# kamenbliznashki/chexpert

Measured on AMD Instinct MI355X. Metric: images/sec fwd+bwd DenseNet121 320x320 bf16 (per-GPU rate in config.images_per_sec_per_gpu), higher is better.
Workload: dtype bf16; 1 GPU; densenet121 bf16 1xMI355X 320x320 bs=256 per GPU, U-Ones labels (BASELINE configs[1]); 14 classes; random-init weights, synthetic uint8 X-rays; per_gpu_batch=256, global_batch=256, parallelism=dp1, rccl_ranks=1, capture_failed=0, launch=hipGraph replay

## Files before the change

### chexpert_amd/csrc/conv_gemm.hip

```cpp
#include "common.h"

namespace {

constexpr int BM = 128;
constexpr int BK = 32;
constexpr int PITCH = 80;
constexpr int A_BYTES = BM * PITCH;

template <int BN>
struct Geo {
  static constexpr int WAVES_N = (BN >= 64) ? 2 : 1;
  static constexpr int WAVES_M = 4 / WAVES_N;
  static constexpr int TM = BM / (WAVES_M * 32);
  static constexpr int TN = BN / (WAVES_N * 32);
  static constexpr int B_BYTES = BN * PITCH;
  static constexpr int STAGE = A_BYTES + B_BYTES;
  static constexpr int EPITCH = BN + 4;
  static constexpr int EPI_BYTES = 64 * EPITCH * 4;
  static constexpr int MAIN_BYTES = (2 * STAGE > EPI_BYTES) ? 2 * STAGE : EPI_BYTES;
};

template <int PRO>
struct NCoef {
  static constexpr int v = (PRO == CX_PRO_NONE) ? 0 : (PRO == CX_PRO_AFFINE_RELU ? 2 : 3);
};

template <int BN, int PRO, int MODE, int EPI>
__global__ __launch_bounds__(256) void conv_gemm_kernel(const CxConv p, const int M, const int n_tiles) {
  using G = Geo<BN>;
  constexpr int NSRC = (MODE == CX_MODE_POOL2) ? 4 : 1;
  extern __shared__ __attribute__((aligned(16))) char smem[];
  float* coef = reinterpret_cast<float*>(smem);
  char* tiles = smem + NCoef<PRO>::v * p.K * 4;

  const int tid = threadIdx.x;
  const int lane = tid & 63;
  const int wave = tid >> 6;
  const int wm = wave / G::WAVES_N, wn = wave % G::WAVES_N;
  const int wgid = xcd_remap(blockIdx.x, gridDim.x);
  const int mt = wgid / n_tiles, nt = wgid % n_tiles;
  const int n0 = nt * BN;

  if (PRO != CX_PRO_NONE) {
    for (int i = tid; i < p.K; i += 256) {
      coef[i] = p.pa[i];
      coef[p.K + i] = p.pb[i];
      if (PRO == CX_PRO_AFFINE2) coef[2 * p.K + i] = p.pc[i];
    }
  }

  const int qa = tid & 3;
  int rb[2], riy[2], rix[2];
  bool rvalid[2];
#pragma unroll
  for (int i = 0; i < 2; ++i) {
    const int m = mt * BM + (tid >> 2) + 64 * i;
    rvalid[i] = m < M;
    const int mm = rvalid[i] ? m : 0;
    const int hw = p.Ho * p.Wo;
    rb[i] = mm / hw;
    const int rem = mm - rb[i] * hw;
    const int oy = rem / p.Wo, ox = rem - oy * p.Wo;
    if (MODE == CX_MODE_CONV) {
      riy[i] = oy * p.stride - p.pad;
      rix[i] = ox * p.stride - p.pad;
    } else if (MODE == CX_MODE_POOL2) {
      riy[i] = 2 * oy;
      rix[i] = 2 * ox;
    } else {
      riy[i] = 2 * oy - 3;
      rix[i] = 2 * ox - 4 + 2 * qa;
    }
  }
  const int kpt = (MODE == CX_MODE_STEM) ? 1 : (p.K + BK - 1) / BK;
  const int taps = (MODE == CX_MODE_STEM) ? 7 : p.kh * p.kw;
  const int nsteps = taps * kpt;
  const bf16* __restrict__ X = reinterpret_cast<const bf16*>(p.x);
  const bf16* __restrict__ X2 = reinterpret_cast<const bf16*>(p.x2);
  const bf16* __restrict__ Wp = reinterpret_cast<const bf16*>(p.w);

  uint4 ra[2][NSRC], ra2[2], rbw[2];
  bool av[2], wv[2] = {false, false};

  const int ts_sh = p.tstride > 1 ? 1 : 0;
  const int cdil = p.dil > 1 ? p.dil : 1;
  int q_tap = 0, q_kc = 0, q_dy = 0, q_dx = 0, w_kc = 0;
  auto issue_loads = [&](int s) {
    (void)s;
    const int tap = q_tap, kc = q_kc;
    const int dy = (MODE == CX_MODE_CONV) ? q_dy * cdil : tap;
    const int dx = (MODE == CX_MODE_CONV) ? q_dx * cdil : 0;
    w_kc = kc;
#pragma unroll
    for (int i = 0; i < 2; ++i) {
      if (MODE == CX_MODE_STEM) {
        const int iy = riy[i] + dy, ix = rix[i];
        av[i] = rvalid[i] & (iy >= 0) & (iy < p.H) & (ix >= 0) & (ix < p.W);
        const int cy = av[i] ? iy : 0, cx = av[i] ? ix : 0;
        ra[i][0] = *reinterpret_cast<const uint4*>(X + ((size_t)(rb[i] * p.H + cy) * p.W + cx) * 4);
      } else if (MODE == CX_MODE_POOL2) {
        av[i] = rvalid[i];
#pragma unroll
        for (int a = 0; a < 4; ++a) {
          const size_t pix = (size_t)(rb[i] * p.H + riy[i] + (a >> 1)) * p.W + rix[i] + (a & 1);
          ra[i][a] = *reinterpret_cast<const uint4*>(X + pix * p.ldx + kc * BK + qa * 8);
        }
      } else {
        int iy = riy[i] + dy, ix = rix[i] + dx;
        bool ok = rvalid[i] & (iy >= 0) & (ix >= 0) & (((iy | ix) & ts_sh) == 0);
        iy >>= ts_sh;
        ix >>= ts_sh;
        const bool kok = kc * BK + qa * 8 < p.K;
// ... 32 lines not shown
    const int tap = 0, kc = w_kc;
    char* A = tiles + buf * G::STAGE;
    char* Bt = A + A_BYTES;
    const int c0 = kc * BK + qa * 8;
#pragma unroll
    for (int i = 0; i < 2; ++i) {
      U128 o;
      if (!av[i]) {
        o.u = make_uint4(0, 0, 0, 0);
      } else if (PRO == CX_PRO_NONE) {
        o.u = ra[i][0];
      } else if (PRO == CX_PRO_AFFINE_RELU) {
        float acc[8];
#pragma unroll
        for (int j = 0; j < 8; ++j) acc[j] = 0.f;
#pragma unroll
        for (int a = 0; a < NSRC; ++a) {
          const uint32_t w4[4] = {ra[i][a].x, ra[i][a].y, ra[i][a].z, ra[i][a].w};
#pragma unroll
          for (int j = 0; j < 4; ++j) {
            acc[2 * j] += fmaxf(fmaf(cx_bf_lo(w4[j]), coef[c0 + 2 * j], coef[p.K + c0 + 2 * j]), 0.f);
            acc[2 * j + 1] += fmaxf(fmaf(cx_bf_hi(w4[j]), coef[c0 + 2 * j + 1], coef[p.K + c0 + 2 * j + 1]), 0.f);
          }
        }
        {
          const float sc_ = NSRC == 4 ? 0.25f : 1.f;
          o.u = make_uint4(cx_packbf(acc[0] * sc_, acc[1] * sc_), cx_packbf(acc[2] * sc_, acc[3] * sc_), cx_packbf(acc[4] * sc_, acc[5] * sc_),
                           cx_packbf(acc[6] * sc_, acc[7] * sc_));
        }
      } else {
        o.u = cx_affine2_8(ra[i][0], ra2[i], coef + c0, coef + p.K + c0, coef + 2 * p.K + c0);
      }
      *reinterpret_cast<uint4*>(A + ((tid >> 2) + 64 * i) * PITCH + qa * 16) = o.u;
    }
#pragma unroll
    for (int i = 0; i < 2; ++i) {
      const int nb = (tid >> 2) + 64 * i;
      if (nb < BN) *reinterpret_cast<uint4*>(Bt + nb * PITCH + qa * 16) = wv[i] ? rbw[i] : make_uint4(0, 0, 0, 0);
    }
    (void)tap;
  };

  f32x16 acc[G::TM][G::TN];
#pragma unroll
  for (int i = 0; i < G::TM; ++i)
#pragma unroll
    for (int j = 0; j < G::TN; ++j)
#pragma unroll
      for (int r = 0; r < 16; ++r) acc[i][j][r] = 0.f;

  issue_loads(0);
  __syncthreads();
  write_stage(0, 0);
  __syncthreads();

  const int lrow = lane & 31, lh = lane >> 5;
  for (int s = 0; s < nsteps; ++s) {
    const int buf = s & 1;
    if (s + 1 < nsteps) issue_loads(s + 1);
    const char* A = tiles + buf * G::STAGE;
    const char* Bt = A + A_BYTES;
#pragma unroll
    for (int kk = 0; kk < 2; ++kk) {
      bf16x8 af[G::TM], bfr[G::TN];
#pragma unroll
      for (int i = 0; i < G::TM; ++i)
// ... 107 lines not shown
            const float du = (fmaf(xu, esc[2 * j + 1], esh[2 * j + 1]) > 0.f) ? v[2 * j + 1] : 0.f;
            s1[2 * j] += dl;
            s1[2 * j + 1] += du;
            s2[2 * j] += dl * (xl - emu[2 * j]) * er[2 * j];
            s2[2 * j + 1] += du * (xu - emu[2 * j + 1]) * er[2 * j + 1];
            w4[j] = cx_packbf(fmaf(escale[2 * j], dl, cx_bf_lo(ow[j])), fmaf(escale[2 * j + 1], du, cx_bf_hi(ow[j])));
          }
          o.u = make_uint4(w4[0], w4[1], w4[2], w4[3]);
        }
        *reinterpret_cast<uint4*>(Y + (size_t)m * p.ldy + nch) = o.u;
      }
    }
    __syncthreads();
  }

  if (want_stats) {
#pragma unroll
    for (int j = 0; j < 8; ++j) {
#pragma unroll
      for (int d = CPR; d < 64; d <<= 1) {
        s1[j] += __shfl_xor(s1[j], d);
        s2[j] += __shfl_xor(s2[j], d);
      }
    }
    float* scratch = reinterpret_cast<float*>(tiles);
    wg_stat_begin<4>(scratch, BN, tid, 256);
    if (lane < CPR) {
#pragma unroll
      for (int j = 0; j < 8; ++j) wg_stat_put(scratch, BN, wave, cq * 8 + j, s1[j], s2[j]);
    }
    wg_stat_end<4>(scratch, BN, tid, 256, p.stat_sum, p.stat_sq, p.stat_det, p.stat_det ? mt : (int)blockIdx.x, p.stat_replicas,
                   p.stat_rstride, n0, p.N);
  }
}

template <int BN, int PRO, int MODE, int EPI>
int launch(const CxConv& p, hipStream_t st) {
  using G = Geo<BN>;
  const long long M = (long long)p.B * p.Ho * p.Wo;
  const int m_tiles = (int)((M + BM - 1) / BM);
  const int n_tiles = (p.N + BN - 1) / BN;
  const size_t smem = (size_t)NCoef<PRO>::v * p.K * 4 + G::MAIN_BYTES + 2 * BN * 4;
  if (smem > 160 * 1024) return CX_ESHAPE;
  if (const int e = stat_rows_check(p, m_tiles)) return e;
  static bool attr_set = false;
  if (!attr_set && smem > 64 * 1024) {
    (void)hipFuncSetAttribute(reinterpret_cast<const void*>(&conv_gemm_kernel<BN, PRO, MODE, EPI>),
                        hipFuncAttributeMaxDynamicSharedMemorySize, 160 * 1024);
    attr_set = true;
  }
  CX_KTAG("conv_gemm_kernel<%d, %d, %d, %d>", BN, PRO, MODE, EPI);
  hipLaunchKernelGGL((conv_gemm_kernel<BN, PRO, MODE, EPI>), dim3(m_tiles * n_tiles), dim3(256), smem, st, p, (int)M,
                     n_tiles);
  return launch_status();
}

template <int PRO, int MODE, int EPI>
int launch_bn(const CxConv& p, hipStream_t st) {
  if (p.N % 128 == 0) return launch<128, PRO, MODE, EPI>(p, st);
  if (p.N == 32) return launch<32, PRO, MODE, EPI>(p, st);
  return launch<64, PRO, MODE, EPI>(p, st);
}

}

int cx_try_pc_fwd(const CxConv& p, hipStream_t st, bool* handled);
int cx_try_ring_fwd(const CxConv& p, hipStream_t st, bool* handled);
int cx_try_strip_fwd(const CxConv& p, hipStream_t st, bool* handled);
int cx_try_ring_dgrad(const CxConv& p, hipStream_t st, bool* handled);
int cx_try_strip_dgrad(const CxConv& p, hipStream_t st, bool* handled);
int cx_try_pw_dgrad(const CxConv& p, hipStream_t st, bool* handled);
int cx_try_pw_fwd(const CxConv& p, hipStream_t st, bool* handled);
int cx_try_pw_fwdk(const CxConv& p, hipStream_t st, bool* handled);
int cx_try_pw_xs(const CxConv& p, hipStream_t st, bool* handled);
int cx_try_stem_fwd(const CxConv& p, hipStream_t st, bool* handled);
int cx_conv_gemm_f32(const CxConv& p, hipStream_t st);
int cx_try_conv_mm(const CxConv& p, hipStream_t st, bool* handled);

thread_local int cx_tl_stat_rows = 0;
thread_local int cx_tl_pro_out = 0;
thread_local char cx_tl_kernel[112] = "";
extern "C" const char* cx_last_kernel(void) { return cx_tl_kernel; }
// ... 80 lines not shown
      if (handled) return rc;
      rc = cx_try_ring_fwd(p, st, &handled);
      if (handled) return rc;
      rc = cx_try_strip_fwd(p, st, &handled);
      if (handled) return rc;
      rc = cx_try_ring_dgrad(p, st, &handled);
      if (handled) return rc;
      rc = cx_try_strip_dgrad(p, st, &handled);
      if (handled) return rc;
      rc = cx_try_pw_dgrad(p, st, &handled);
      if (handled) return rc;
      rc = cx_try_pw_fwd(p, st, &handled);
      if (handled) return rc;
      rc = cx_try_pw_fwdk(p, st, &handled);
      if (handled) return rc;
      rc = cx_try_pw_xs(p, st, &handled);
      if (handled) return rc;
      rc = cx_try_conv_mm(p, st, &handled);
      if (handled) return rc;
    }
    if (p.epilogue == CX_EPI_STORE) {
      if (p.prologue == CX_PRO_NONE) return launch_bn<CX_PRO_NONE, CX_MODE_CONV, CX_EPI_STORE>(p, st);
      if (p.prologue == CX_PRO_AFFINE_RELU) return launch_bn<CX_PRO_AFFINE_RELU, CX_MODE_CONV, CX_EPI_STORE>(p, st);
      if (p.prologue == CX_PRO_AFFINE2) return launch_bn<CX_PRO_AFFINE2, CX_MODE_CONV, CX_EPI_STORE>(p, st);
    } else if (p.epilogue == CX_EPI_MASK) {
      if (p.prologue == CX_PRO_AFFINE2) return launch_bn<CX_PRO_AFFINE2, CX_MODE_CONV, CX_EPI_MASK>(p, st);
      if (p.prologue == CX_PRO_NONE) return launch_bn<CX_PRO_NONE, CX_MODE_CONV, CX_EPI_MASK>(p, st);
    }
    return CX_EUNSUPPORTED;
  }
  if (p.mode == CX_MODE_POOL2) {
    if (p.prologue != CX_PRO_AFFINE_RELU || p.epilogue != CX_EPI_STORE) return CX_EUNSUPPORTED;
    if ((p.H & 1) || (p.W & 1) || p.Ho != p.H / 2 || p.Wo != p.W / 2 || p.ldx < p.K) return CX_ESHAPE;
    return launch_bn<CX_PRO_AFFINE_RELU, CX_MODE_POOL2, CX_EPI_STORE>(p, st);
  }
  if (p.mode == CX_MODE_STEM) {
    if (p.prologue != CX_PRO_NONE || p.epilogue != CX_EPI_STORE) return CX_EUNSUPPORTED;
    if (p.K != 32 || (p.W & 1) || p.Ho != (p.H + 6 - 7) / 2 + 1 || p.Wo != (p.W + 6 - 7) / 2 + 1) return CX_ESHAPE;
    {
      bool handled = false;
      const int rc = cx_try_stem_fwd(p, st, &handled);
      if (handled) return rc;
    }
    return launch_bn<CX_PRO_NONE, CX_MODE_STEM, CX_EPI_STORE>(p, st);
  }
  return CX_EUNSUPPORTED;
}
```

### chexpert_amd/models/densenet.py

```python
import os
from collections import OrderedDict

import torch
import torch.nn as nn

from .. import ops
from ._fused import FusedEngine, FusedNet, _Vec, flatten


class _FusedOnly:
    def forward(self, *a, **k):
        raise RuntimeError("chexpert_amd: this sub-module only holds parameters; call the parent model "
                           "(the fused HIP schedule).  There is no module-by-module fallback.")


class Conv2dParams(_FusedOnly, nn.Conv2d):
    pass


class BatchNorm2dParams(_FusedOnly, nn.BatchNorm2d):
    pass


class ReLUMarker(_FusedOnly, nn.ReLU):
# ... 116 lines not shown


class _Workspace:

    def __init__(self, eng, B, H, W, dev):
        bf, u8 = eng.dtype, torch.uint8
        self.key = (B, H, W)
        self.B, self.H, self.W = B, H, W
        g = eng.growth
        e = lambda *s, dtype=bf: torch.empty(*s, dtype=dtype, device=dev)
        if eng.cifar:
            self.x8 = e(B, H, W, 8)
            h, w = H, W
            self.c0 = e(B, h, w, eng.c_init)
            self.dz0 = None
            self.amax = None
        else:
            self.x4 = e(B, H, W, 4)
            h, w = H // 2, W // 2
            self.c0 = e(B, h, w, eng.c_init)
            self.dz0 = None
            h, w = h // 2, w // 2
            self.amax = e(B, h, w, eng.c_init, dtype=u8)
        self.buf, self.gbuf, self.y1, self.hw = [], [], [], []
        for bi, (c_in, n_layers) in enumerate(eng.blocks):
            ct = c_in + n_layers * g
            self.buf.append(torch.zeros(B, h, w, ct, dtype=bf, device=dev) if eng.cifar else e(B, h, w, ct))
            self.gbuf.append(None)
            self.y1.append([e(B, h, w, eng.mid) for _ in range(n_layers)])
            self.hw.append((h, w))
            h, w = h // 2, w // 2
        self.dz2 = None
        self.dpool = None
        self.aa = {}
        f32 = torch.float32
        for bi, (c_in, n_layers) in enumerate(eng.blocks[:-1]):
            aa = getattr(eng.model.features, "transition%d" % (bi + 1)).conv
            if not isinstance(aa, AAConv2d):
                continue
            ct = c_in + n_layers * g
            (hh, wh), (ho, wo) = self.hw[bi], self.hw[bi + 1]
            if (ho, wo) != tuple(aa.input_dims):
                raise RuntimeError("AAConv2d was built for %s feature maps, the input gives %s (relative tables are size-bound, "
                                   "attn_aug_conv.py:38-41)" % (tuple(aa.input_dims), (ho, wo)))
            T = type("AAWs", (), {})()
            T.stat = torch.zeros(2, B * ct, dtype=f32, device=dev)
            T.coef = torch.zeros(2, B * ct, dtype=f32, device=dev)
            T.A = e(B, hh, wh, ct)
            T.QKV = e(B, ho, wo, 2 * aa.dk + aa.dv)
            T.O = torch.empty(B, ho * wo, aa.dv, dtype=f32, device=dev)
            T.LSE = torch.empty(B * aa.nh, ho * wo, dtype=f32, device=dev)
            T.bwd = None
            self.aa[bi] = T
        self.pooled = torch.empty(B, eng.c_final, dtype=torch.float32, device=dev)
        self.logits = torch.empty(B, eng.n_classes, dtype=torch.float32, device=dev)
        self.vec = torch.zeros(eng.vec_size, dtype=torch.float32, device=dev)
        self.ones = torch.ones(max(eng.mid, 64, eng.c_init), dtype=torch.float32, device=dev)
        self.zeros = torch.zeros(max(eng.growth, 8), dtype=torch.float32, device=dev)
        self.slab = torch.empty(2, eng.SLAB, dtype=torch.float32, device=dev) if eng.det else None

    def v(self, slot):
        off, n = slot
        return self.vec[off:off + n]

    def alloc_backward(self, eng, dev):
        if self.dz0 is not None:
# ... 32 lines not shown
        if sub is not None:
            a, b = (a[0] + sub[0], sub[1]), (b[0] + sub[0], sub[1])
        return dict(stat_sum=ws.v(a), stat_sq=ws.v(b), stat_replicas=self.stat_replicas, stat_rstride=slots[0][1])

    def _ew(self, ws, slots, C, rows=None):
        if self.det:
            return ws.slab[0], ws.slab[1], rows or min(self.EW_ROWS, self.SLAB // C)
        return ws.v(slots[0]), ws.v(slots[1]), 0

    def _sc(self, ws, slots, C, rows, copies=True):
        if self.det:
            return ws.slab[0], ws.slab[1], rows, C
        return ws.v(slots[0]), ws.v(slots[1]), self.stat_replicas if copies else 1, slots[0][1] if copies else 0

    def __init__(self, model):
        super().__init__(model)
        f = model.features
        self.growth = model.growth_rate
        self.mid = getattr(model, "_mid", None) or model.bn_size * model.growth_rate
        self.c_init = f.conv0.out_channels
        self.cifar = not hasattr(f, "pool0")
        self.blocks = []
        c = self.c_init
        for n_layers in model.block_config:
            self.blocks.append((c, n_layers))
            c = c + n_layers * self.growth
            if len(self.blocks) != len(model.block_config):
                c = getattr(f, "denseblock%d" % (len(self.blocks) + 1)).denselayer1.norm1.num_features
        self.c_final = c
        self.stat_replicas = 16
        self.drop_rate = float(getattr(model, "drop_rate", 0.0))
        self.drop_seed = None
        self.pair_bwd = os.environ.get("CHEXPERT_PAIR_BWD", "0")
        self._w2_items = []
        self._plan_vectors()

    def _plan_vectors(self):
        V = _Vec()
        s = {}
        R = self.stat_replicas
        take_r = lambda n: (V.take(n * R)[0], n)
        s["st0"] = [V.take(self.c_init) for _ in range(2)]
        s["bst"] = [[take_r(c + n * self.growth) for _ in range(2)] for c, n in self.blocks]
        s["yst"] = [[[take_r(self.mid) for _ in range(2)] for _ in range(n)] for _, n in self.blocks]
        self.fwd_zero = (0, V.n)
        s["n0"] = [V.take(self.c_init) for _ in range(4)]
        s["bmr"] = [[V.take(c + n * self.growth) for _ in range(2)] for c, n in self.blocks]
        s["n1"] = [[[V.take(c + i * self.growth) for _ in range(2)] for i in range(n)] for c, n in self.blocks]
        s["n2"] = [[[V.take(self.mid) for _ in range(4)] for _ in range(n)] for _, n in self.blocks]
        s["nt"] = [[V.take(c + n * self.growth) for _ in range(2)] for c, n in self.blocks]
        b0 = V.n
        s["S0"] = [V.take(self.c_init) for _ in range(2)]
        s["S1"] = [[[take_r(c + i * self.growth) for _ in range(2)] for i in range(n)] for c, n in self.blocks]
        s["S2"] = [[[take_r(self.mid) for _ in range(2)] for _ in range(n)] for _, n in self.blocks]
        s["St"] = [[V.take(c + n * self.growth) for _ in range(2)] for c, n in self.blocks]
        s["AB"] = [[V.take(c + n * self.growth) for _ in range(2)] for c, n in self.blocks]
        self.bwd_zero = (b0, V.n - b0)
        s["ql"] = [[[V.take(self.growth) for _ in range(3)] for _ in range(n)] for _, n in self.blocks]
        s["pl"] = [[[V.take(self.mid) for _ in range(3)] for _ in range(n)] for _, n in self.blocks]
        s["q"] = [V.take(max(self.mid, self.c_init, max(c for c, _ in self.blocks))) for _ in range(3)]
        s["p"] = [V.take(max(self.mid, self.c_init)) for _ in range(3)]
        s["dpooled"] = V.take(0)
        self.slots = s
        self.vec_size = V.n

    def bind(self, dev):
        if self.bound(dev):
            return
        m = self.model
        if m.classifier.in_features != self.c_final:
            raise RuntimeError("classifier.in_features must be %d" % self.c_final)
        self.bind_params(dev)
        self.n_classes = m.classifier.out_features
        f = m.features
        self.plan_packing([mod for mod in f.modules() if isinstance(mod, nn.Conv2d) and mod is not f.conv0], stem=f.conv0,
                          stem_layout=not self.cifar)
        self.eye = torch.eye(self.c_init, dtype=self.dtype, device=dev).reshape(-1) if self.cifar else None

    def _new_workspace(self, B, H, W):
        return _Workspace(self, B, H, W, self.device)

    def _bn(self, ws, stats, count, bn, out_slots, C_, train, mean_slot=None, rstd_slot=None):
        sc, sh = ws.v(out_slots[0])[:C_], ws.v(out_slots[1])[:C_]
        mean = ws.v(mean_slot)[:C_] if mean_slot is not None else None
        rstd = ws.v(rstd_slot)[:C_] if rstd_slot is not None else None
        if train:
            mom = bn.momentum if bn.momentum is not None else 0.1
            ssum, ssq, reps, rstride = stats
            ops.bn_coef(ssum, ssq, count, bn.weight, bn.bias, bn.eps, mom,
                        bn.running_mean if bn.track_running_stats else None,
                        bn.running_var if bn.track_running_stats else None, sc, sh, mean, rstd, C_, replicas=reps, rstride=rstride)
        else:
            ops.bn_coef_eval(bn.running_mean, bn.running_var, bn.weight, bn.bias, bn.eps, sc, sh, mean, rstd, C_)

    def _bn_block(self, ws, bi, cin, count, bn, out_slots, train, fresh):
        s = self.slots
        bmean, brstd = s["bmr"][bi]
        if not train:
            return self._bn(ws, None, count, bn, out_slots, cin, False, bmean, brstd)
        if not self.det:
            bsum, bsq = s["bst"][bi]
            return self._bn(ws, (ws.v(bsum), ws.v(bsq), self.stat_replicas, bsum[1]), count, bn, out_slots, cin, True, bmean, brstd)
        mom = bn.momentum if bn.momentum is not None else 0.1
        ops.bn_coef_moments(ws.v(bmean)[:cin], ws.v(brstd)[:cin], count, bn.weight, bn.bias, bn.eps, mom,
                            bn.running_mean if bn.track_running_stats else None, bn.running_var if bn.track_running_stats else None,
                            ws.v(out_slots[0])[:cin], ws.v(out_slots[1])[:cin], cin, fresh)

    def forward(self, x, train, record=False):
        m, f, s = self.model, self.model.features, self.slots
        det = self.det and train
# ... 53 lines not shown
                cin = c0 + li * g_
                n1, n2 = s["n1"][bi][li], s["n2"][bi][li]
                self._bn_block(ws, bi, cin, cnt, layer.norm1, n1, train, fresh)
                yst = s["yst"][bi][li]
                y1 = ws.y1[bi][li]
                rows = ops.conv_gemm(buf[..., :cin], self.w_fwd(layer.conv1), y1, N=self.mid, prologue=ops.PRO_AFFINE_RELU,
                                     pa=ws.v(n1[0]), pb=ws.v(n1[1]), **sp(yst, self.mid))
                self._bn(ws, self._sc(ws, yst, self.mid, rows) if train else None, cnt, layer.norm2, n2[:2], self.mid, train, n2[2],
                         n2[3])
                rows = ops.conv_gemm(y1, self.w_fwd(layer.conv2), buf[..., cin:cin + g_], N=g_, kh=3, kw=3, pad=1,
                                     prologue=ops.PRO_AFFINE_RELU, pa=ws.v(n2[0]), pb=ws.v(n2[1]),
                                     **({} if drop else sp(s["bst"][bi], g_, (cin, g_))))
                if drop:
                    rows = ops.dropout_slice_fwd(buf[..., cin:cin + g_], self.drop_rate, self.drop_seed, bi * 256 + li, ws.slab[0],
                                                 ws.slab[1], stat_rows=min(self.EW_ROWS, self.SLAB // g_))
                if det:
                    fresh = (ws.slab[0], ws.slab[1], rows, g_, cin, g_)
            ct = c0 + n_layers * g_
            nt = s["nt"][bi]
            if bi != nb - 1 and isinstance(getattr(f, "transition%d" % (bi + 1)).conv, AAConv2d):
                bmean, brstd = s["bmr"][bi]
                if train and det:
                    ops.bn_coef_moments(ws.v(bmean)[:ct], ws.v(brstd)[:ct], cnt, None, None, 1e-5, 0.0, None, None, None, None, ct, fresh)
                elif train:
                    bsum, bsq = s["bst"][bi]
                    ops.bn_coef(ws.v(bsum), ws.v(bsq), cnt, None, None, 1e-5, 0.0, None, None, None, None, ws.v(bmean), ws.v(brstd), ct,
                                replicas=self.stat_replicas, rstride=bsum[1])
                st = (lambda a: ws.v(a)) if train else (lambda a: None)
                fresh = self._aa_forward(ws, bi, getattr(f, "transition%d" % (bi + 1)).conv, st, det)
            elif bi != nb - 1:
                tr = getattr(f, "transition%d" % (bi + 1))
                self._bn_block(ws, bi, ct, cnt, tr.norm, nt, train, fresh)
                cn = self.blocks[bi + 1][0]
                rows = ops.conv_gemm(buf, self.w_fwd(tr.conv), ws.buf[bi + 1][..., :cn], N=cn, mode=ops.MODE_POOL2,
                                     prologue=ops.PRO_AFFINE_RELU, pa=ws.v(nt[0]), pb=ws.v(nt[1]),
                                     **sp(s["bst"][bi + 1], cn, (0, cn)))
                if det:
                    fresh = (ws.slab[0], ws.slab[1], rows, cn, 0, cn)
            else:
                self._bn_block(ws, bi, ct, cnt, f.norm5, nt, train, fresh)
                ops.head_fwd(buf, ws.v(nt[0]), ws.v(nt[1]), m.classifier.weight, m.classifier.bias, ws.pooled, ws.logits)
        if train:
            m._nbt_pending += 1
        return ws

    def _cifar_stem(self, ws, x, train, sp):
        f, s = self.model.features, self.slots
        B, H, W = ws.B, ws.H, ws.W
        ops.nchw3_to_nhwc8(x.contiguous().float(), ws.x8)
        rows = ops.conv_gemm(ws.x8, self.w_fwd(f.conv0), ws.c0, N=self.c_init, kh=5, kw=5, pad=2, **sp(None, self.c_init))
        st0 = (ws.slab[0], ws.slab[1], rows, self.c_init) if train else None
        self._bn(ws, st0, B * H * W, f.norm0, s["n0"][:2], self.c_init, train, s["n0"][2], s["n0"][3])
        self._stem_rows = ops.conv_gemm(ws.c0, self.eye, ws.buf[0][..., :self.c_init], N=self.c_init, prologue=ops.PRO_AFFINE_RELU,
                                        pa=ws.v(s["n0"][0]), pb=ws.v(s["n0"][1]), **sp(None, self.c_init))

    def _aa_forward(self, ws, bi, aa, st, det=False):
        s = self.slots
        buf, nxt, T = ws.buf[bi], ws.buf[bi + 1], ws.aa[bi]
        B, h, w, ct = buf.shape
        cc = aa.conv.out_channels
        cout = cc + aa.dv
        ops.stats_bc(buf, T.stat[0], T.stat[1])
        ops.bn_coef(T.stat[0], T.stat[1], h * w, None, None, 1e-5, 0.0, None, None, T.coef[0], T.coef[1], None, None, B * ct)
        ops.affine_relu_bc(buf, T.coef[0], T.coef[1], T.A)
        nsum, nsq = s["bst"][bi + 1]
        fresh = None
        if det:
            rows = ops.conv_gemm(T.A, self.w_fwd(aa.conv), nxt[..., :cc], N=cc, kh=3, kw=3, stride=2, pad=1, **self._sp(ws, None, cc))
            nmean, nrstd = s["bmr"][bi + 1]
# ... 156 lines not shown
        layer = self._layer(bi, li)
        h, w = ws.hw[bi]
        buf, gbuf, y1 = ws.buf[bi], ws.gbuf[bi], ws.y1[bi][li]
        cin = self.blocks[bi][0] + li * self.growth
        n1, S1, (bmean, brstd), (A, Bc) = s["n1"][bi][li], s["S1"][bi][li], s["bmr"][bi], s["AB"][bi]
        pa, pb, pc = pabc
        rows = ops.conv_gemm(dz2, self.w_bwd(layer.conv1), gbuf[..., :cin], N=cin, prologue=ops.PRO_AFFINE2, x2=y1, pa=pa,
                             pb=pb, pc=pc, epilogue=ops.EPI_MASK, ex=buf[..., :cin], e_sc=v(n1[0]), e_sh=v(n1[1]),
                             e_mu=v(bmean)[:cin], e_r=v(brstd)[:cin], e_scale=v(n1[0]), accumulate=True,
                             fused_dw=G(layer.conv1.weight) if fused else None, **self._sp(ws, S1, cin))
        red1 = self._sc(ws, S1, cin, rows)
        if not fused:
            ops.conv_wgrad(dz2, buf[..., :cin], G(layer.conv1.weight), g_prologue=ops.PRO_AFFINE2, g2=y1, ga=pa, gb=pb,
                           gc=pc, x_prologue=ops.PRO_AFFINE_RELU, pa=v(n1[0]), pb=v(n1[1]))
        self.bn_bwd_coef(ws, layer.norm1, red1[0], red1[1], ws.B * h * w, layer.norm1.weight, v(bmean), v(brstd), G(layer.norm1.weight),
                         G(layer.norm1.bias), v(A), v(Bc), None, None, None, cin, replicas=red1[2], rstride=red1[3],
                         q=self._slice_q(ws, bi, li - 1))
        done(layer.norm1.weight)

    def _transition_backward(self, ws, bi, done):
        s, v, G = self.slots, ws.v, self.grad_of
        qa, qb, qc, _, c0 = self._slice_q(ws, bi, -1)
        gs, xs = ws.gbuf[bi][..., :c0], ws.buf[bi][..., :c0]
        B, (h, w), (ph, pw) = ws.B, ws.hw[bi], ws.hw[bi - 1]
        pc0, pn = self.blocks[bi - 1]
        cprev = pc0 + pn * self.growth
        tr = getattr(self.model.features, "transition%d" % bi)
        pbuf, pg = ws.buf[bi - 1], ws.gbuf[bi - 1]
        nt, (pmean, prstd), (pA, pB), St = s["nt"][bi - 1], s["bmr"][bi - 1], s["AB"][bi - 1], s["St"][bi - 1]
        dpool = ws.dpool[:B * h * w * cprev].view(B, h, w, cprev)
        ops.conv_gemm(gs, self.w_bwd(tr.conv), dpool, N=cprev, prologue=ops.PRO_AFFINE2, x2=xs, pa=qa, pb=qb, pc=qc)
        rows = ops.unpool2_mask(dpool, pbuf, v(nt[0]), v(nt[1]), v(pmean), v(prstd), v(nt[0]), pg, *self._ew(ws, St, cprev))
        sred = self._sc(ws, St, cprev, rows, copies=False)
        ops.conv_wgrad(gs, pbuf, G(tr.conv.weight), mode=ops.MODE_POOL2, g_prologue=ops.PRO_AFFINE2, g2=xs, ga=qa, gb=qb,
                       gc=qc, x_prologue=ops.PRO_AFFINE_RELU, pa=v(nt[0]), pb=v(nt[1]))
        self.bn_bwd_coef(ws, tr.norm, sred[0], sred[1], B * ph * pw, tr.norm.weight, v(pmean), v(prstd), G(tr.norm.weight),
                         G(tr.norm.bias), v(pA), v(pB), None, None, None, cprev, replicas=sred[2], rstride=sred[3],
                         q=self._slice_q(ws, bi - 1, pn - 1))
        done(tr.norm.weight)

    def _stem_backward(self, ws, dx):
        f, s, v, G = self.model.features, self.slots, ws.v, self.grad_of
        ci = self.c_init
        qa, qb, qc = self._slice_q(ws, 0, -1)[:3]
        gs, xs = ws.gbuf[0][..., :ci], ws.buf[0][..., :ci]
        n0, S0 = s["n0"], s["S0"]
        rows = ops.bnrelu_maxpool_bwd(ws.c0, v(n0[0]), v(n0[1]), v(n0[2]), v(n0[3]), ws.amax, gs, xs, qa, qb, qc, ws.dz0,
                                      *self._ew(ws, S0, ci))
        sred = self._sc(ws, S0, ci, rows, copies=False)
        pa, pb, pc = (v(t)[:ci] for t in s["p"])
        self.bn_bwd_coef(ws, f.norm0, sred[0], sred[1], ws.B * (ws.H // 2) * (ws.W // 2), f.norm0.weight, v(n0[2]), v(n0[3]),
                         G(f.norm0.weight), G(f.norm0.bias), None, None, pa, pb, pc, ci, replicas=sred[2], rstride=sred[3])
        ops.conv_wgrad(ws.dz0, ws.x4, G(f.conv0.weight), mode=ops.MODE_STEM, g_prologue=ops.PRO_AFFINE2, g2=ws.c0, ga=pa, gb=pb,
                       gc=pc)
        if dx is not None:
            ops.stem_input_grad(ws.dz0, ws.c0, pa, pb, pc, f.conv0.weight, dx, stride=2, pad=3)

    def _cifar_stem_backward(self, ws, dx):
        f, s, v, G = self.model.features, self.slots, ws.v, self.grad_of
        ci = self.c_init
        qa, qb, qc = self._slice_q(ws, 0, -1)[:3]
        gs, xs = ws.gbuf[0][..., :ci], ws.buf[0][..., :ci]
        n0, S0 = s["n0"], s["S0"]
        rows = ops.conv_gemm(gs, self.eye, ws.dz0, N=ci, prologue=ops.PRO_AFFINE2, x2=xs, pa=qa, pb=qb, pc=qc,
                             epilogue=ops.EPI_MASK, ex=ws.c0, e_sc=v(n0[0]), e_sh=v(n0[1]), e_mu=v(n0[2]), e_r=v(n0[3]),
                             e_scale=ws.ones[:ci], **self._sp(ws, S0, ci))
        sred = self._sc(ws, S0, ci, rows)
        pa, pb, pc = (v(t)[:ci] for t in s["p"])
# ... 313 lines not shown
```

### chexpert_amd/ops.py

```python
import os

import torch

from . import _lib as L
from ._lib import (EPI_JOIN, EPI_MASK, EPI_STORE, MODE_CONV, MODE_POOL2, MODE_STEM, PRO_AFFINE2, PRO_AFFINE_RELU, PRO_JOIN, PRO_NONE,
                   CxConv, CxWgrad, check, lib, ptr, require_cuda, stream_ptr)
import ctypes as C


def _nhwc(t):
    assert t.dtype in (torch.bfloat16, torch.float32) and t.dim() == 4, "expected a bf16 (or fp32-mode) NHWC tensor"
    B, H, W, Cc = t.shape
    sb, sh, sw, sc = t.stride()
    assert sc == 1 and sh == W * sw and sb == H * sh, "NHWC slice must be dense in (B,H,W) with a channel pitch"
    return B, H, W, Cc, sw


def _dense(t, like=None):
    B, H, W, Cc, ld = _nhwc(t)
    assert ld == Cc, "this kernel takes dense NHWC tensors (no channel pitch)"
    assert like is None or (t.shape == like.shape and t.dtype == like.dtype), "NHWC operands of one launch share shape and storage type"
    return B, H, W, Cc


# ... 170 lines not shown
                 pc=None, x2=None, epilogue=EPI_STORE, stat_sum=None, stat_sq=None, ex=None, e_sc=None, e_sh=None,
                 e_mu=None, e_r=None, e_scale=None, accumulate=False, K=None, tstride=1, stat_replicas=1, stat_rstride=0,
                 stat_det=False, pro_out=None, emask=None, x3=None, po_lo=None, po_mask=None, dil=1, hint=None):
    require_cuda(x, w_packed, y)
    p = CxConv()
    p.kernel_hint = KERNEL_HINT if hint is None else hint
    B, H, W, Cx, ldx = _nhwc(x)
    By, Ho, Wo, Cy, ldy = _nhwc(y)
    assert By == B and Cy == N
    p.x, p.w, p.y = ptr(x), ptr(w_packed), ptr(y)
    p.B, p.H, p.W, p.Ho, p.Wo = B, H, W, Ho, Wo
    p.K = (32 if mode == MODE_STEM else Cx) if K is None else K
    p.N = N
    p.ldx, p.ldy = ldx, ldy
    p.kh, p.kw, p.stride, p.pad = kh, kw, stride, pad
    p.prologue, p.mode, p.epilogue, p.accumulate = prologue, mode, epilogue, int(accumulate)
    p.dil = dil
    p.tstride = tstride
    p.pa, p.pb, p.pc = ptr(pa), ptr(pb), ptr(pc)
    if x2 is not None:
        assert x2.shape == x.shape
        p.x2, p.ldx2 = ptr(x2), _nhwc(x2)[4]
    p.stat_sum, p.stat_sq = ptr(stat_sum), ptr(stat_sq)
    p.stat_replicas, p.stat_rstride, p.stat_det = stat_replicas, stat_rstride, int(bool(stat_det))
    p.dtype = 1 if x.dtype == torch.float32 else 0
    for t_ in (w_packed, y, x2, ex):
        assert t_ is None or t_.dtype == x.dtype, "all tensors of one convolution share the storage type"
    if ex is not None:
        assert ex.shape == y.shape
        p.ex, p.ldex = ptr(ex), _nhwc(ex)[4]
    p.e_sc, p.e_sh, p.e_mu, p.e_r, p.e_scale = ptr(e_sc), ptr(e_sh), ptr(e_mu), ptr(e_r), ptr(e_scale)
    if pro_out is not None:
        require_cuda(pro_out)
        assert pro_out.dtype == x.dtype and tuple(pro_out.shape) == tuple(x.shape)
        p.pro_out, p.ldpo = ptr(pro_out), _nhwc(pro_out)[4]
    if emask is not None:
        require_cuda(emask)
        assert emask.dtype == torch.uint8 and emask.is_contiguous() and emask.numel() * 8 == B * Ho * Wo * N
        p.emask = ptr(emask)
    if prologue == PRO_JOIN:
        assert x2 is not None and pro_out is not None and x.is_contiguous() and x2.is_contiguous()
        for t_, n_ in ((x3, x.numel()), (po_lo, x.numel()), (po_mask, x.numel() // 8)):
            if t_ is not None:
                require_cuda(t_)
                assert t_.dtype in (torch.int8, torch.uint8) and t_.is_contiguous() and t_.numel() == n_
        p.x3, p.po_lo, p.po_mask = ptr(x3), ptr(po_lo), ptr(po_mask)
    p._keep = (x, w_packed, y, pa, pb, pc, x2, stat_sum, stat_sq, ex, e_sc, e_sh, e_mu, e_r, e_scale, pro_out, emask, x3, po_lo, po_mask)
    return p


def conv_wgrad(g, x, dw, *, kh=1, kw=1, stride=1, pad=0, mode=MODE_CONV, g_prologue=PRO_NONE, g2=None, ga=None, gb=None,
               gc=None, x_prologue=PRO_NONE, pa=None, pb=None, splits=0, K=None, dil=1, hint=None):
    require_cuda(g, x, dw)
    p = CxWgrad()
    p.kernel_hint = KERNEL_HINT if hint is None else hint
    p.dil = dil
    B, Ho, Wo, N, ldg = _nhwc(g)
    Bx, H, W, Cx, ldx = _nhwc(x)
    assert Bx == B and dw.dtype == torch.float32 and dw.is_contiguous()
    p.g, p.x, p.dw = ptr(g), ptr(x), ptr(dw)
    p.B, p.H, p.W, p.Ho, p.Wo = B, H, W, Ho, Wo
    p.K = (32 if mode == MODE_STEM else Cx) if K is None else K
    p.N = N
    p.ldg, p.ldx = ldg, ldx
    if g2 is not None:
        assert g2.shape == g.shape
        p.g2, p.ldg2 = ptr(g2), _nhwc(g2)[4]
    p.ga, p.gb, p.gc, p.pa, p.pb = ptr(ga), ptr(gb), ptr(gc), ptr(pa), ptr(pb)
    p.kh, p.kw, p.stride, p.pad = kh, kw, stride, pad
    p.g_prologue, p.x_prologue, p.mode, p.splits = g_prologue, x_prologue, mode, splits
    p.dtype = 1 if g.dtype == torch.float32 else 0
    assert x.dtype == g.dtype and (g2 is None or g2.dtype == g.dtype)
    ws, arena, dfr = _wgrad_ws(dw.device)
    if ws is not None:
        p.scratch, p.scratch_floats = ptr(ws), ws.numel()
    check(lib().cx_conv_wgrad(C.byref(p), stream_ptr()), "cx_conv_wgrad")
    _wgrad_used(arena, dfr)


def stem_input_grad(dz, y, pa, pb, pc, w, dx, *, stride, pad):
    require_cuda(dz, y, pa, pb, pc, w, dx)
    B, Ho, Wo, C0, ldz = _nhwc(dz)
    By, Hy, Wy, Cy, ldy = _nhwc(y)
    assert (By, Hy, Wy, Cy) == (B, Ho, Wo, C0) and y.dtype == dz.dtype
    assert w.dtype == torch.float32 and w.is_contiguous() and w.dim() == 4 and w.shape[0] == C0 and w.shape[2] == w.shape[3]
    assert dx.dtype == torch.float32 and dx.is_contiguous() and dx.dim() == 4 and dx.shape[:2] == (B, 3)
    for t in (pa, pb, pc):
        assert t.dtype == torch.float32 and t.is_contiguous() and t.numel() >= C0
    H, W = dx.shape[2], dx.shape[3]
    check(lib().cx_stem_input_grad(ptr(dz), ptr(y), ptr(pa), ptr(pb), ptr(pc), ptr(w), ptr(dx), ldz, ldy, w.shape[1], B, H, W, Ho, Wo, C0,
                                   w.shape[2], stride, pad, 1 if dz.dtype == torch.float32 else 0, stream_ptr()), "cx_stem_input_grad")
    return dx


def conv3x3_wgrad_batch(items):
    n = len(items)
    if n == 0:
        return True
    g0, x0 = items[0][0], items[0][1]
    if n > L.WGRAD_BATCH_MAX or g0.dtype != torch.bfloat16:
        return False
    p, bt = CxWgrad(), L.CxWgradBatch()
    B, H, W, N, ldg = _nhwc(g0)
    _, _, _, K, ldx = _nhwc(x0)
    p.B, p.H, p.W, p.Ho, p.Wo, p.K, p.N = B, H, W, H, W, K, N
    p.ldg, p.ldx = ldg, ldx
    p.kh, p.kw, p.stride, p.pad = 3, 3, 1, 1
    p.g_prologue, p.x_prologue, p.mode, p.dtype = PRO_NONE, PRO_AFFINE_RELU, MODE_CONV, 0
    for i, (g, x, pa, pb, dw) in enumerate(items):
        require_cuda(g, x, dw)
# ... 673 lines not shown
```

Baseline: 9623 images/sec.

## Save pooled transition activations in forward and reuse them for transition weight grad

The forward transition conv (affine+ReLU, 2x2 avgpool, 1x1 GEMM) gets a side-output kernel variant that writes the pooled, activated input tile to a saved buffer, written only by the first N-tile. In backward, transition weight-gradient uses this saved pooled tensor with a plain 1x1 wgrad, avoiding recomputing affine/ReLU/pool over the 4x larger pre-pool activation. The exchange is extra forward stores and workspace memory for the pooled buffers, plus a fallback path when shape conditions fail.

```diff
diff --git a/chexpert_amd/csrc/conv_gemm.hip b/chexpert_amd/csrc/conv_gemm.hip
--- a/chexpert_amd/csrc/conv_gemm.hip
+++ b/chexpert_amd/csrc/conv_gemm.hip
@@ -25,8 +25,8 @@
   static constexpr int v = (PRO == CX_PRO_NONE) ? 0 : (PRO == CX_PRO_AFFINE_RELU ? 2 : 3);
 };
 
-template <int BN, int PRO, int MODE, int EPI>
-__global__ __launch_bounds__(256) void conv_gemm_kernel(const CxConv p, const int M, const int n_tiles) {
+template <int BN, int PRO, int MODE, int EPI, bool SIDE>
+__device__ __forceinline__ void conv_gemm_body(const CxConv& p, const int M, const int n_tiles) {
   using G = Geo<BN>;
   constexpr int NSRC = (MODE == CX_MODE_POOL2) ? 4 : 1;
   extern __shared__ __attribute__((aligned(16))) char smem[];
@@ -78,6 +78,7 @@
   const bf16* __restrict__ X = reinterpret_cast<const bf16*>(p.x);
   const bf16* __restrict__ X2 = reinterpret_cast<const bf16*>(p.x2);
   const bf16* __restrict__ Wp = reinterpret_cast<const bf16*>(p.w);
+  bf16* __restrict__ PO = (SIDE && nt == 0) ? reinterpret_cast<bf16*>(p.pro_out) : nullptr;
 
   uint4 ra[2][NSRC], ra2[2], rbw[2];
   bool av[2], wv[2] = {false, false};
@@ -176,6 +177,9 @@
         o.u = cx_affine2_8(ra[i][0], ra2[i], coef + c0, coef + p.K + c0, coef + 2 * p.K + c0);
       }
       *reinterpret_cast<uint4*>(A + ((tid >> 2) + 64 * i) * PITCH + qa * 16) = o.u;
+      if (SIDE) {
+        if (PO && av[i]) *reinterpret_cast<uint4*>(PO + (size_t)(mt * BM + (tid >> 2) + 64 * i) * p.ldpo + c0) = o.u;
+      }
     }
 #pragma unroll
     for (int i = 0; i < 2; ++i) {
@@ -349,6 +353,16 @@
     wg_stat_end<4>(scratch, BN, tid, 256, p.stat_sum, p.stat_sq, p.stat_det, p.stat_det ? mt : (int)blockIdx.x, p.stat_replicas,
                    p.stat_rstride, n0, p.N);
   }
+}
+
+template <int BN, int PRO, int MODE, int EPI>
+__global__ __launch_bounds__(256) void conv_gemm_kernel(const CxConv p, const int M, const int n_tiles) {
+  conv_gemm_body<BN, PRO, MODE, EPI, false>(p, M, n_tiles);
+}
+
+template <int BN>
+__global__ __launch_bounds__(256) void conv_gemm_pool2_side_kernel(const CxConv p, const int M, const int n_tiles) {
+  conv_gemm_body<BN, CX_PRO_AFFINE_RELU, CX_MODE_POOL2, CX_EPI_STORE, true>(p, M, n_tiles);
 }
 
 template <int BN, int PRO, int MODE, int EPI>
@@ -365,6 +379,18 @@
     (void)hipFuncSetAttribute(reinterpret_cast<const void*>(&conv_gemm_kernel<BN, PRO, MODE, EPI>),
                         hipFuncAttributeMaxDynamicSharedMemorySize, 160 * 1024);
     attr_set = true;
+  }
+  if constexpr (MODE == CX_MODE_POOL2) if (p.pro_out) {
+    static bool side_attr_set = false;
+    if (!side_attr_set && smem > 64 * 1024) {
+      (void)hipFuncSetAttribute(reinterpret_cast<const void*>(&conv_gemm_pool2_side_kernel<BN>), hipFuncAttributeMaxDynamicSharedMemorySize,
+                                160 * 1024);
+      side_attr_set = true;
+    }
+    CX_KTAG("conv_gemm_pool2_side_kernel<%d>", BN);
+    hipLaunchKernelGGL((conv_gemm_pool2_side_kernel<BN>), dim3(m_tiles * n_tiles), dim3(256), smem, st, p, (int)M, n_tiles);
+    cx_tl_pro_out = 1;
+    return launch_status();
   }
   CX_KTAG("conv_gemm_kernel<%d, %d, %d, %d>", BN, PRO, MODE, EPI);
   hipLaunchKernelGGL((conv_gemm_kernel<BN, PRO, MODE, EPI>), dim3(m_tiles * n_tiles), dim3(256), smem, st, p, (int)M,
@@ -511,6 +537,7 @@
   if (p.mode == CX_MODE_POOL2) {
     if (p.prologue != CX_PRO_AFFINE_RELU || p.epilogue != CX_EPI_STORE) return CX_EUNSUPPORTED;
     if ((p.H & 1) || (p.W & 1) || p.Ho != p.H / 2 || p.Wo != p.W / 2 || p.ldx < p.K) return CX_ESHAPE;
+    if (p.pro_out && ((p.ldpo % 8) || p.ldpo < p.K || !aligned16(p.pro_out))) return CX_EALIGN;
     return launch_bn<CX_PRO_AFFINE_RELU, CX_MODE_POOL2, CX_EPI_STORE>(p, st);
   }
   if (p.mode == CX_MODE_STEM) {
diff --git a/chexpert_amd/models/densenet.py b/chexpert_amd/models/densenet.py
--- a/chexpert_amd/models/densenet.py
+++ b/chexpert_amd/models/densenet.py
@@ -172,6 +172,11 @@
             h, w = h // 2, w // 2
         self.dz2 = None
         self.dpool = None
+        self.tp = [None] * len(eng.blocks)
+        self.tp_valid = [False] * len(eng.blocks)
+        for bi in range(len(eng.blocks) - 1):
+            if eng._pool_once_ok(B, self.hw[bi + 1], self.buf[bi].shape[3], self.buf[bi + 1].shape[3], bi):
+                self.tp[bi] = e(B, *self.hw[bi + 1], self.buf[bi].shape[3])
         self.aa = {}
         f32 = torch.float32
         for bi, (c_in, n_layers) in enumerate(eng.blocks[:-1]):
@@ -270,6 +275,7 @@
         self.drop_rate = float(getattr(model, "drop_rate", 0.0))
         self.drop_seed = None
         self.pair_bwd = os.environ.get("CHEXPERT_PAIR_BWD", "0")
+        self.pool_once = os.environ.get("CHEXPERT_POOL_ONCE", "1") != "0"
         self._w2_items = []
         self._plan_vectors()
 
@@ -314,6 +320,11 @@
         self.plan_packing([mod for mod in f.modules() if isinstance(mod, nn.Conv2d) and mod is not f.conv0], stem=f.conv0,
                           stem_layout=not self.cifar)
         self.eye = torch.eye(self.c_init, dtype=self.dtype, device=dev).reshape(-1) if self.cifar else None
+
+    def _pool_once_ok(self, B, hw, ct, ct_next, bi):
+        if not self.pool_once or self.dtype != torch.bfloat16 or self.cifar or self._aa_transition(bi + 1) is not None:
+            return False
+        return ops.wide_wgrad_1x1_ok(B * hw[0] * hw[1], self.blocks[bi + 1][0], ct, max(ct, ct_next))
 
     def _new_workspace(self, B, H, W):
         return _Workspace(self, B, H, W, self.device)
@@ -433,9 +444,11 @@
                 tr = getattr(f, "transition%d" % (bi + 1))
                 self._bn_block(ws, bi, ct, cnt, tr.norm, nt, train, fresh)
                 cn = self.blocks[bi + 1][0]
+                tp = ws.tp[bi] if (train or record) and self.pool_once else None
                 rows = ops.conv_gemm(buf, self.w_fwd(tr.conv), ws.buf[bi + 1][..., :cn], N=cn, mode=ops.MODE_POOL2,
-                                     prologue=ops.PRO_AFFINE_RELU, pa=ws.v(nt[0]), pb=ws.v(nt[1]),
+                                     prologue=ops.PRO_AFFINE_RELU, pa=ws.v(nt[0]), pb=ws.v(nt[1]), pro_out=tp,
                                      **sp(s["bst"][bi + 1], cn, (0, cn)))
+                ws.tp_valid[bi] = tp is not None and ops.last_pro_out()
                 if det:
                     fresh = (ws.slab[0], ws.slab[1], rows, cn, 0, cn)
             else:
@@ -658,8 +671,8 @@
         ops.conv_gemm(gs, self.w_bwd(tr.conv), dpool, N=cprev, prologue=ops.PRO_AFFINE2, x2=xs, pa=qa, pb=qb, pc=qc)
         rows = ops.unpool2_mask(dpool, pbuf, v(nt[0]), v(nt[1]), v(pmean), v(prstd), v(nt[0]), pg, *self._ew(ws, St, cprev))
         sred = self._sc(ws, St, cprev, rows, copies=False)
-        ops.conv_wgrad(gs, pbuf, G(tr.conv.weight), mode=ops.MODE_POOL2, g_prologue=ops.PRO_AFFINE2, g2=xs, ga=qa, gb=qb,
-                       gc=qc, x_prologue=ops.PRO_AFFINE_RELU, pa=v(nt[0]), pb=v(nt[1]))
+        ops.transition_wgrad(gs, xs, qa, qb, qc, pbuf, v(nt[0]), v(nt[1]), ws.tp[bi - 1] if ws.tp_valid[bi - 1] else None,
+                             G(tr.conv.weight))
         self.bn_bwd_coef(ws, tr.norm, sred[0], sred[1], B * ph * pw, tr.norm.weight, v(pmean), v(prstd), G(tr.norm.weight),
                          G(tr.norm.bias), v(pA), v(pB), None, None, None, cprev, replicas=sred[2], rstride=sred[3],
                          q=self._slice_q(ws, bi - 1, pn - 1))
diff --git a/chexpert_amd/ops.py b/chexpert_amd/ops.py
--- a/chexpert_amd/ops.py
+++ b/chexpert_amd/ops.py
@@ -226,7 +226,8 @@
     p.e_sc, p.e_sh, p.e_mu, p.e_r, p.e_scale = ptr(e_sc), ptr(e_sh), ptr(e_mu), ptr(e_r), ptr(e_scale)
     if pro_out is not None:
         require_cuda(pro_out)
-        assert pro_out.dtype == x.dtype and tuple(pro_out.shape) == tuple(x.shape)
+        want = (B, Ho, Wo, Cx) if mode == MODE_POOL2 else tuple(x.shape)
+        assert pro_out.dtype == x.dtype and tuple(pro_out.shape) == want
         p.pro_out, p.ldpo = ptr(pro_out), _nhwc(pro_out)[4]
     if emask is not None:
         require_cuda(emask)
@@ -270,6 +271,21 @@
         p.scratch, p.scratch_floats = ptr(ws), ws.numel()
     check(lib().cx_conv_wgrad(C.byref(p), stream_ptr()), "cx_conv_wgrad")
     _wgrad_used(arena, dfr)
+
+
+def wide_wgrad_1x1_ok(M, N, K, ld):
+    return M % 64 == 0 and N % 128 == 0 and K % 8 == 0 and K >= 64 and M * ld * 2 < (1 << 32)
+
+
+def transition_wgrad(g, g2, ga, gb, gc, x, pa, pb, pooled, dw):
+    B, Ho, Wo, N, ldg = _nhwc(g)
+    if pooled is not None and g.dtype == torch.bfloat16:
+        K, ldp = _nhwc(pooled)[3:]
+        if wide_wgrad_1x1_ok(B * Ho * Wo, N, K, max(ldg, _nhwc(g2)[4], ldp)):
+            conv_wgrad(g, pooled, dw, g_prologue=PRO_AFFINE2, g2=g2, ga=ga, gb=gb, gc=gc)
+            return True
+    conv_wgrad(g, x, dw, mode=MODE_POOL2, g_prologue=PRO_AFFINE2, g2=g2, ga=ga, gb=gb, gc=gc, x_prologue=PRO_AFFINE_RELU, pa=pa, pb=pb)
+    return False
 
 
 def stem_input_grad(dz, y, pa, pb, pc, w, dx, *, stride, pad):
```

Measured after the change: 9660 images/sec, median of 2. Within noise of the previous version (+0.4%).
